# dongzhuoyao/uspace

Hardware: AMD Instinct MI355X
Metric: images/sec, U-ViT-L 256 latent FM sampling (50 ODE steps, bs64) @1/2/4/8 GPU (higher is better)
Workload: dtype bf16

## Files before the change

include/uspace_hip.h:

```cpp
#ifndef USPACE_HIP_H
#define USPACE_HIP_H

#include <stddef.h>
#include <stdint.h>

#ifdef __cplusplus
extern "C" {
#endif

#define USPACE_ABI_VERSION 11

#define USPACE_OK 0
#define USPACE_ERR_ARG (-1)
#define USPACE_ERR_LAUNCH (-2)
#define USPACE_ERR_WORKSPACE (-3)

typedef void* uspace_stream_t;

#define USPACE_API __attribute__((visibility("default")))

USPACE_API int uspace_abi_version(void);


#define USPACE_EPI_BIAS 1
// ... 21 lines not shown
    const float* colsum;
    float* c_out;
    int norm_dim;
    float eps;
    const float* row_add;
    const float* col_add;
    void* split_ws;
    size_t split_ws_bytes;
    void* sk_ws;
    size_t sk_ws_bytes;
    void* sk_counters;
} uspace_gemm_ext;
USPACE_API size_t uspace_gemm_split_ws_bytes(int M, int N, int K);
USPACE_API size_t uspace_gemm_sk_ws_bytes(int M, int N, int K);
#define USPACE_GEMM_SK_COUNTERS 256
USPACE_API int uspace_gemm_set_sk(int mode);
USPACE_API int uspace_gemm_get_sk(void);
USPACE_API int uspace_gemm_bf16_ext(const uint16_t* A, int lda, const uint16_t* A2, int lda2, int K1,
                                    const uint16_t* W, int ldw, int M, int N, int K, int epi_flags,
                                    const float* bias, const float* resid_in, int ld_resid,
                                    float* out_f32, int ld_f32, uint16_t* out_bf16, int ld_bf16,
                                    const uspace_gemm_ext* ext, uspace_stream_t stream);
USPACE_API int uspace_fold_layernorm(const float* W, const float* gamma, const float* beta, const float* bias, uint16_t* Wf,
                                     float* bias_out, float* colsum, int N, int K, uspace_stream_t stream);
USPACE_API int uspace_center_rows(const float* x, uint16_t* xc, float* c, float* part, int M, int D, uspace_stream_t stream);
USPACE_API int uspace_uvit_set_ln_fold(int mode);
USPACE_API int uspace_uvit_get_ln_fold(void);
USPACE_API int uspace_gemm_part_slots(int M, int N);
USPACE_API int uspace_gemm_part_slots_k(int M, int N, int K);

USPACE_API int uspace_gemm_tile_choice(int M, int N, int* split_rows);
USPACE_API int uspace_gemm_plan(int M, int N, int* out);
USPACE_API int uspace_gemm_plan_k(int M, int N, int K, int producer, int* out);

USPACE_API int uspace_gemm_slabs_bf16(const uint16_t* A, int lda, const uint16_t* W, int ldw, int M, int N, int K1,
                                      int n_slab, const int* row_shift, int epi_flags, const float* bias,
                                      const float* resid_in, int ld_resid, float* out_f32, int ld_f32,
                                      uint16_t* out_bf16, int ld_bf16, uspace_stream_t stream);

USPACE_API int uspace_layernorm_f32_bf16(const float* x, const float* gamma, const float* beta, uint16_t* y,
                              int M, int D, float eps, uspace_stream_t stream);

USPACE_API int uspace_attention_bf16(const uint16_t* qkv, const float* key_scale, uint16_t* out,
                          int B, int L, int H, uspace_stream_t stream);
USPACE_API int uspace_attention_plan(int B, int L, int H, int scaled, int* out);

USPACE_API int uspace_attention_long_bf16(const uint16_t* qkv, const float* key_scale, uint16_t* out,
                                          int B, int L, int H, uspace_stream_t stream);
USPACE_API int uspace_attention_long_plan(int B, int L, int H, int scaled, int* out);

USPACE_API int uspace_attention_wide_bf16(const uint16_t* q, const uint16_t* k, const uint16_t* v, int ld,
                                          uint16_t* out, int ld_out, int B, int N, int C, float scale,
                                          uspace_stream_t stream);
USPACE_API int uspace_attention_wide_plan(int B, int N, int C, int* out);

USPACE_API int uspace_attention_map_bf16(const uint16_t* qkv, float* out, int B, int L, int H,
                                         int q0, int nq, int k0, int nk, uspace_stream_t stream);

USPACE_API int uspace_embed_tokens(const float* img, const float* t, int t_stride, const float* extra, int n_extra,
                        int time_first, const float* patch_w, const float* patch_b, const float* pos,
                        float* tok, uint16_t* tok_bf16, int B, int C, int S, int p, int D,
                        uspace_stream_t stream);

USPACE_API int uspace_output_head(const float* tok, int L, int extras, const float* norm_g, const float* norm_b,
                       const float* dec_w, const float* dec_b, const float* conv_w, const float* conv_b,
                       float* scratch, float* out, int B, int C, int S, int p, int D, float eps,
// ... 301 lines not shown
```

uspace_amd/_hip.py:

```python
import ctypes
import os

import torch

_HERE = os.path.dirname(os.path.abspath(__file__))
_DEFAULT_LIB = os.path.join(_HERE, "libuspace_hip.so")
LIB_PATH = os.environ.get("USPACE_HIP_LIB") or _DEFAULT_LIB

EPI_BIAS, EPI_GELU, EPI_RESIDUAL, EPI_OUT_F32, EPI_OUT_BF16 = 1, 2, 4, 8, 16
EPI_CEN_OUT, EPI_LN_IN, EPI_RANK1 = 32, 64, 128

ABI_VERSION = 11

_ERR = {-1: "USPACE_ERR_ARG", -2: "USPACE_ERR_LAUNCH", -3: "USPACE_ERR_WORKSPACE"}


class UspaceHipError(RuntimeError):
    pass


class UvitConfig(ctypes.Structure):
    _fields_ = [(n, ctypes.c_int) for n in (
        "img_size", "patch_size", "in_chans", "embed_dim", "depth", "num_heads", "mlp_hidden",
        "n_extra", "clip_dim", "time_first")]
# ... 31 lines not shown
    _fields_ = [("input_size", ctypes.c_int), ("blocks", ctypes.c_int * 4), ("se", ctypes.c_int)]


class GemmExt(ctypes.Structure):
    _fields_ = [("row_c", ctypes.c_void_p), ("out_cen", ctypes.c_void_p), ("ld_cen", ctypes.c_int),
                ("part_out", ctypes.c_void_p), ("part_in", ctypes.c_void_p), ("np_in", ctypes.c_int),
                ("colsum", ctypes.c_void_p), ("c_out", ctypes.c_void_p), ("norm_dim", ctypes.c_int), ("eps", ctypes.c_float),
                ("row_add", ctypes.c_void_p), ("col_add", ctypes.c_void_p),
                ("split_ws", ctypes.c_void_p), ("split_ws_bytes", ctypes.c_size_t),
                ("sk_ws", ctypes.c_void_p), ("sk_ws_bytes", ctypes.c_size_t), ("sk_counters", ctypes.c_void_p)]


_P, _I, _L, _F, _SZ = ctypes.c_void_p, ctypes.c_int, ctypes.c_long, ctypes.c_float, ctypes.c_size_t
_D = ctypes.c_double

SIGNATURES = {
    "uspace_abi_version": (_I, []),
    "uspace_gemm_bf16": (_I, [_P, _I, _P, _I, _I, _P, _I, _I, _I, _I, _I, _P, _P, _I, _P, _I, _P, _I, _P]),
    "uspace_gemm_bf16_ext": (_I, [_P, _I, _P, _I, _I, _P, _I, _I, _I, _I, _I, _P, _P, _I, _P, _I, _P, _I,
                                  ctypes.POINTER(GemmExt), _P]),
    "uspace_gemm_part_slots": (_I, [_I, _I]),
    "uspace_gemm_part_slots_k": (_I, [_I, _I, _I]),
    "uspace_gemm_split_ws_bytes": (_SZ, [_I, _I, _I]),
    "uspace_gemm_sk_ws_bytes": (_SZ, [_I, _I, _I]),
    "uspace_gemm_set_sk": (_I, [_I]),
    "uspace_gemm_get_sk": (_I, []),
    "uspace_fold_layernorm": (_I, [_P, _P, _P, _P, _P, _P, _P, _I, _I, _P]),
    "uspace_center_rows": (_I, [_P, _P, _P, _P, _I, _I, _P]),
    "uspace_uvit_set_ln_fold": (_I, [_I]),
    "uspace_uvit_get_ln_fold": (_I, []),
    "uspace_gemm_tile_choice": (_I, [_I, _I, ctypes.POINTER(_I)]),
    "uspace_gemm_plan": (_I, [_I, _I, ctypes.POINTER(_I)]),
    "uspace_gemm_plan_k": (_I, [_I, _I, _I, _I, ctypes.POINTER(_I)]),
    "uspace_gemm_slabs_bf16": (_I, [_P, _I, _P, _I, _I, _I, _I, _I, ctypes.POINTER(_I), _I, _P, _P, _I, _P, _I, _P, _I, _P]),
    "uspace_layernorm_f32_bf16": (_I, [_P, _P, _P, _P, _I, _I, _F, _P]),
    "uspace_attention_bf16": (_I, [_P, _P, _P, _I, _I, _I, _P]),
    "uspace_attention_plan": (_I, [_I, _I, _I, _I, ctypes.POINTER(_I)]),
    "uspace_attention_long_bf16": (_I, [_P, _P, _P, _I, _I, _I, _P]),
    "uspace_attention_long_plan": (_I, [_I, _I, _I, _I, ctypes.POINTER(_I)]),
    "uspace_attention_wide_bf16": (_I, [_P, _P, _P, _I, _P, _I, _I, _I, _I, _F, _P]),
    "uspace_attention_wide_plan": (_I, [_I, _I, _I, ctypes.POINTER(_I)]),
    "uspace_attention_map_bf16": (_I, [_P, _P, _I, _I, _I, _I, _I, _I, _I, _P]),
    "uspace_embed_tokens": (_I, [_P, _P, _I, _P, _I, _I, _P, _P, _P, _P, _P, _I, _I, _I, _I, _I, _P]),
    "uspace_output_head": (_I, [_P, _I, _I, _P, _P, _P, _P, _P, _P, _P, _P, _I, _I, _I, _I, _I, _F, _P]),
    "uspace_add_broadcast": (_I, [_P, _P, _P, _F, _I, _L, _P]),
    "uspace_add_broadcast_rows": (_I, [_P, _P, _P, _F, _P, _I, _L, _P]),
    "uspace_cast_f32_bf16": (_I, [_P, _P, _L, _P]),
    "uspace_cfg_combine": (_I, [_P, _P, _F, _P, _I, _L, _P]),
    "uspace_direction_accumulate": (_I, [_P, _P, _P, _P, _I, _L, _I, _P]),
    "uspace_center_cols_f32": (_I, [_P, _P, _I, _L, _P]),
    "uspace_gram_f64": (_I, [_P, _P, _I, _L, _P]),
    "uspace_project_rows_f64": (_I, [_P, _P, _P, _I, _I, _L, _P]),
    "uspace_normalize_rows_signed": (_I, [_P, _I, _L, _P]),
    "uspace_ode_combine": (_I, [_P, _P, ctypes.POINTER(_P), ctypes.POINTER(_F), _I, _L, _P]),
    "uspace_ode_error_norm": (_I, [_P, _P, ctypes.POINTER(_P), ctypes.POINTER(_F), _I, _F, _F, _L, _P, _P, _P]),
    "uspace_uvit_num_params": (_I, [ctypes.POINTER(UvitConfig)]),
    "uspace_uvit_param_numel": (_L, [ctypes.POINTER(UvitConfig), _I]),
    "uspace_uvit_weight_bytes": (_SZ, [ctypes.POINTER(UvitConfig)]),
    "uspace_uvit_workspace_bytes": (_SZ, [ctypes.POINTER(UvitConfig), _I]),
    "uspace_uvit_pack_weights": (_I, [ctypes.POINTER(UvitConfig), ctypes.POINTER(_P), _I, _P, _SZ, _P]),
    "uspace_uvit_forward": (_I, [ctypes.POINTER(UvitConfig), _P, _P, _SZ, ctypes.POINTER(UvitIO), _I, _P]),
    "uspace_uvit_forward_maps": (_I, [ctypes.POINTER(UvitConfig), _P, _P, _SZ, ctypes.POINTER(UvitIO), _I, _I, _I, _I, _I, _P, _P]),
    "uspace_uvit_cfg_workspace_bytes": (_SZ, [ctypes.POINTER(UvitConfig), _I]),
    "uspace_uvit_forward_cfg": (_I, [ctypes.POINTER(UvitConfig), _P, _P, _SZ, ctypes.POINTER(UvitIO), _I, _P, _I, _F, _P, _P, _P]),
    "uspace_uvit_forward_tap": (_I, [ctypes.POINTER(UvitConfig), _P, _P, _SZ, ctypes.POINTER(UvitIO), _I, _I, _P, _P]),
    "uspace_uvit_graph_create": (_I, [ctypes.POINTER(UvitConfig), _P, _P, _SZ, ctypes.POINTER(UvitIO), _I, _P,
# ... 483 lines not shown
```

uspace_amd/csrc/gemm.hip:

```cpp
#include <algorithm>
#include <atomic>
#include <type_traits>
#include <vector>

#include "common.h"
#include "gemm_args.h"

namespace {

using namespace usgemm;


#ifndef USPACE_LAB
#define USPACE_LAB 0
#endif
constexpr size_t sk_slab_bytes(int BM, int BN, bool xtra) { return (size_t)((BM / 16) * (BN / 16) + (xtra ? BN / 16 : 0)) * 1024; }
constexpr double TALL_COST = 0.60;
constexpr int ROW_BYTES = 128;

template <int WM, int XN, int TN>
__device__ __forceinline__ bf16x8 pick_w(const bf16x8 (&wf)[TN], int wm, int j) {
    if constexpr (WM == 4) {
        const bf16x8 a = wf[j], b = wf[XN + j], c = wf[2 * XN + j], d = wf[3 * XN + j];
        const bf16x8 lo = (wm & 1) ? b : a, hi = (wm & 1) ? d : c;
// ... 7 lines not shown

template <int WM, int XN, int TN>
__device__ __forceinline__ f32x4 pick_b(const f32x4 (&b)[TN], int wm, int j) {
    if constexpr (WM == 4) {
        const f32x4 a = b[j], b1 = b[XN + j], c = b[2 * XN + j], d = b[3 * XN + j];
        const f32x4 lo = (wm & 1) ? b1 : a, hi = (wm & 1) ? d : c;
        return (wm & 2) ? hi : lo;
    }
    f32x4 r = b[j];
#pragma unroll
    for (int w = 1; w < WM; ++w) r = (wm == w) ? b[w * XN + j] : r;
    return r;
}

__device__ __forceinline__ uint4 widen_pair(uint2 a, uint2 b) {
    const auto rx = __builtin_amdgcn_permlane16_swap(a.x, b.x, false, false);
    const auto ry = __builtin_amdgcn_permlane16_swap(a.y, b.y, false, false);
    return make_uint4(rx[0], ry[0], rx[1], ry[1]);
}

__device__ __forceinline__ int lds_off(int r, int c) { return r * ROW_BYTES + ((c ^ ((r >> 1) & 7)) << 4); }

template <int N>
__device__ __forceinline__ void wait_vm() {
    asm volatile("s_waitcnt vmcnt(%0) lgkmcnt(0)" ::"n"(N) : "memory");
}

constexpr int stage_bytes(int BM, int BN, bool xtra) { return (BM + BN + (xtra ? 16 : 0)) * ROW_BYTES; }
constexpr int rowv_bytes(int BM, int flags) { return (flags & (USPACE_EPI_LN_IN | USPACE_EPI_CEN_OUT)) ? (BM + 16) * 8 : 0; }
__device__ __forceinline__ int strip_of_tile_row(int tile_m, int tiles_m) {
    return (tiles_m & 7) == 0 ? (tile_m & 7) * (tiles_m >> 3) + (tile_m >> 3) : tile_m;
}

template <int BM, int BN, int WM, int WN, int FLAGS, bool XTRA, int NST, bool SK, bool OWNER>
__device__ __forceinline__ void gemm_tile(const GemmArgs& g, char* const smem, const int tile_m, const int tile_n, const int sk_tile,
                                          const int sk_split) {
    static_assert(!OWNER || (XTRA && NST == 2 && !SK), "a strip owner's body has the strips and is a two-stage whole-tile form");
    constexpr int THREADS = 64 * WM * WN;
    constexpr int TM = BM / WM / 16;
    constexpr int TN = BN / WN / 16;
    constexpr int HM = TM / 2;
    constexpr int XN = TN / WM;
    constexpr int ROWS_PER_ISSUE = THREADS / 8;
    constexpr int ISSUES_A = BM / ROWS_PER_ISSUE;
    constexpr int ISSUES_W = BN / ROWS_PER_ISSUE;
    constexpr int TILE_A_BYTES = BM * ROW_BYTES;
    constexpr int TILE_W_BYTES = BN * ROW_BYTES;
    constexpr int TILE_X_BYTES = XTRA ? 16 * ROW_BYTES : 0;
    constexpr int STAGE_BYTES = TILE_A_BYTES + TILE_W_BYTES + TILE_X_BYTES;
    static_assert(BM % ROWS_PER_ISSUE == 0 && BN % ROWS_PER_ISSUE == 0, "tile/threads mismatch");
    static_assert(TM % 2 == 0 && TN % WM == 0 && (WM == 2 || WM == 4), "wave tile shape");
    static_assert(NST == 2 || (!XTRA && FLAGS == USPACE_EPI_OUT_F32) || (BM == 64 && BN == 64),
                  "the ring form: raw fp32 partial sums of a K range (K-split), or the 64 x 64 tiles with any epilogue");
    constexpr int IPT = ISSUES_A + ISSUES_W;
    static_assert((NST - 1) * IPT < 64, "vmcnt is a 6-bit counter");
    static_assert(!SK || (NST == 2 && WM * WN == 8), "the in-launch K-split tail is written for the 8-wave two-stage forms (one workgroup per CU)");

    constexpr bool ROWV = (FLAGS & (USPACE_EPI_LN_IN | USPACE_EPI_CEN_OUT)) != 0;
    static_assert(STAGE_BYTES == stage_bytes(BM, BN, XTRA), "the kernel sizes the LDS object with stage_bytes");
    const uint32_t rowv_lds = (uint32_t)(uintptr_t)(US_LDS char*)(smem + NST * STAGE_BYTES);

    const int tid = threadIdx.x;
    const int lane = tid & 63;
    const int wave = __builtin_amdgcn_readfirstlane(tid >> 6);
    const int wm = wave / WN;
    const int wn = wave % WN;

    const int m0 = tile_m * BM;
    const int n0 = tile_n * BN;
    const int m_lim = XTRA ? g.m_main : g.M;
    const int sk = strip_of_tile_row(tile_m, g.tiles_m);
    const int x0 = g.m_main + sk * 16;
    const int xr = (XTRA && sk < g.n_strip) ? (g.M - x0 < 16 ? g.M - x0 : 16) : 0;
    const bool has_x = OWNER || xr > 0;

    const int srow = tid >> 3;
    const int schunk = tid & 7;
    const bf16_t* const gA = g.A;
    const bf16_t* const gA2 = g.A2;
    const bf16_t* const gW = g.W;
    uint32_t a_off[ISSUES_A];
    uint32_t w_off[ISSUES_W];
#pragma unroll
    for (int i = 0; i < ISSUES_A; ++i) {
        const int r = i * ROWS_PER_ISSUE + srow;
        const int c = schunk ^ ((r >> 1) & 7);
        int m = m0 + r;
        m = m < m_lim ? m : m_lim - 1;
        a_off[i] = (uint32_t)(m * g.lda + c * 8) * 2u;
    }
#pragma unroll
    for (int i = 0; i < ISSUES_W; ++i) {
        const int r = i * ROWS_PER_ISSUE + srow;
        const int c = schunk ^ ((r >> 1) & 7);
        int n = n0 + r;
        n = n < g.N ? n : g.N - 1;
        w_off[i] = (uint32_t)(n * g.ldw + c * 8) * 2u;
    }
    uint32_t x_off = 0;
    if constexpr (XTRA) {
        const int r = tid >> 3;
        const int c = schunk ^ ((r >> 1) & 7);
        int m = x0 + (r < xr ? r : 0);
        m = m < g.M ? m : g.M - 1;
        x_off = (uint32_t)(m * g.lda + c * 8) * 2u;
    }
    const int wave_lds_off = wave * 8 * ROW_BYTES;
// ... 28 lines not shown
        char* base = smem + buf * STAGE_BYTES + TILE_A_BYTES;
        const __amdgpu_buffer_rsrc_t rs = __builtin_amdgcn_make_buffer_rsrc((void*)wbase, 0, 0x7fffffff, 0x00020000);
#pragma unroll
        for (int i = 0; i < ISSUES_W; ++i) dma16(rs, w_off[i], base + i * ROWS_PER_ISSUE * ROW_BYTES + wave_lds_off);
    };

    const int fr = lane & 15;
    const int fq = lane >> 4;
    const int a_lds = (wm * (BM / WM) + fr) * ROW_BYTES;
    const int w_lds = TILE_A_BYTES + (wn * (BN / WN) + fr) * ROW_BYTES;
    const int x_lds = TILE_A_BYTES + TILE_W_BYTES + fr * ROW_BYTES;
    const int swz = (fr >> 1) & 7;
    const int c_k0 = ((fq) ^ swz) << 4;
    const int c_k1 = ((4 + fq) ^ swz) << 4;

    f32x4 acc[TM][TN];
    f32x4 xacc[XTRA ? XN : 1];
    if ((FLAGS & USPACE_EPI_RESIDUAL) != 0 && (!SK || sk_split == 0)) {
#pragma unroll
        for (int i = 0; i < TM; ++i) {
            int m = m0 + wm * (BM / WM) + i * 16 + fr;
            m = m < m_lim ? m : m_lim - 1;
#pragma unroll
            for (int j = 0; j < TN; ++j) {
                int n = n0 + wn * (BN / WN) + j * 16 + fq * 4;
                n = n < g.N ? n : g.N - 4;
                acc[i][j] = *(const f32x4*)(g.resid + (size_t)m * g.ld_resid + n);
            }
        }
        if constexpr (XTRA) {
            int m = x0 + (fr < xr ? fr : 0);
            m = m < g.M ? m : g.M - 1;
#pragma unroll
            for (int j = 0; j < XN; ++j) {
                int n = n0 + wn * (BN / WN) + (wm * XN + j) * 16 + fq * 4;
                n = n < g.N ? n : g.N - 4;
                xacc[j] = *(const f32x4*)(g.resid + (size_t)m * g.ld_resid + n);
            }
        }
    } else {
#pragma unroll
        for (int i = 0; i < TM; ++i)
#pragma unroll
            for (int j = 0; j < TN; ++j) acc[i][j] = (f32x4){0.f, 0.f, 0.f, 0.f};
#pragma unroll
        for (int j = 0; j < (XTRA ? XN : 1); ++j) xacc[j] = (f32x4){0.f, 0.f, 0.f, 0.f};
    }

    bf16x8 af0[HM], af1[HM], wf0[TN], wf1[TN], xf0, xf1;

    constexpr bool LN_IN = (FLAGS & USPACE_EPI_LN_IN) != 0, CEN = (FLAGS & USPACE_EPI_CEN_OUT) != 0;
    constexpr bool RK1 = (FLAGS & USPACE_EPI_RANK1) != 0;
    static_assert(!RK1 || (CEN && !LN_IN), "the rank-1 term belongs to a LayerNorm producer (skip_linear)");
    constexpr bool CSV = LN_IN || RK1;
    constexpr bool EARLY_EPI = BM * BN <= 256 * 128;
    f32x4 bias4[TN];
    f32x4 cs4[CSV ? TN : 1];
    auto load_epi_consts = [&]() {
        if constexpr (FLAGS & USPACE_EPI_BIAS) {
#pragma unroll
            for (int j = 0; j < TN; ++j) {
                int n = n0 + wn * (BN / WN) + j * 16 + fq * 4;
                n = n < g.N ? n : g.N - 4;
                bias4[j] = *(const f32x4*)(g.bias + n);
            }
        }
        if constexpr (CSV) {
            const float* const cv = RK1 ? g.col_add : g.colsum;
#pragma unroll
            for (int j = 0; j < TN; ++j) {
                int n = n0 + wn * (BN / WN) + j * 16 + fq * 4;
                n = n < g.N ? n : g.N - 4;
                cs4[j] = *(const f32x4*)(cv + n);
            }
        }
    };

#define LOAD_A(dst, base, mh, ck)                                                                   \
    _Pragma("unroll") for (int i_ = 0; i_ < HM; ++i_)                                               \
        dst[i_] = *(const bf16x8*)((base) + a_lds + ((mh) * HM + i_) * 16 * ROW_BYTES + (ck));
#define LOAD_W(dst, base, ck)                                                                       \
    _Pragma("unroll") for (int j_ = 0; j_ < TN; ++j_)                                               \
        dst[j_] = *(const bf16x8*)((base) + w_lds + j_ * 16 * ROW_BYTES + (ck));
#define LOAD_X(dst, base, ck) if (X_ON) dst = *(const bf16x8*)((base) + x_lds + (ck));
#define MMA(af, wf, mh, ilo, ihi)                                                                   \
    _Pragma("unroll") for (int i_ = (ilo); i_ < (ihi); ++i_)                                        \
        _Pragma("unroll") for (int jj_ = 0; jj_ < TN; ++jj_) {                                      \
            const int j_ = (i_ & 1) ? TN - 1 - jj_ : jj_;                                           \
            acc[(mh) * HM + i_][j_] =                                                               \
                __builtin_amdgcn_mfma_f32_16x16x32_bf16(wf[j_], af[i_], acc[(mh) * HM + i_][j_], 0, 0, 0); \
        }
#define MMA_X(xf, wf)                                                                               \
    if (XTRA && X_ON) {                                                                             \
        _Pragma("unroll") for (int j_ = 0; j_ < XN; ++j_)                                           \
            xacc[j_] = __builtin_amdgcn_mfma_f32_16x16x32_bf16(pick_w<WM, XN>(wf, wm, j_), xf, xacc[j_], 0, 0, 0); \
    }

    const bool X_ON = has_x;
    const int nk = NST > 2 ? g.nk_split : (SK && sk_tile >= 0) ? (sk_split + 1) * (g.K / BK) / g.sk_S - kt0 : g.K / BK;
    float2 pr[ROWV ? 8 : 1];
    float rc_v = 0.f, ra_v = 0.f;
    int rv_m = -1;
    auto fetch_rowv = [&]() {
        static_assert(BM + 16 <= THREADS || !ROWV, "one thread per tile row");
        const int t = tid;
        if (t < BM + (XTRA ? 16 : 0)) {
            const bool strip = t >= BM;
            const int m = strip ? x0 + (t - BM) : m0 + t;
            const bool ok = strip ? ((t - BM) < xr && m < g.M) : (m < m_lim);
            if (ok) {
                rv_m = m;
                if constexpr ((FLAGS & USPACE_EPI_LN_IN) != 0) {
#pragma unroll
                    for (int q = 0; q < 8; ++q)
                        pr[q] = q < g.np_in ? *(const float2*)(g.part_in + ((size_t)m * g.np_in + q) * 2) : make_float2(0.f, 0.f);
                    if (n0 == 0 && g.c_out && sk_split == 0) rc_v = g.row_c[m];
                } else {
                    rc_v = g.row_c[m];
                    if constexpr (RK1) ra_v = g.row_add[m];
                }
            }
        }
    };
    if constexpr (NST > 2) {
        if constexpr (ROWV) fetch_rowv();
        if constexpr (EARLY_EPI) load_epi_consts();
#pragma unroll
        for (int t = 0; t < 2; ++t) {
            stage_a(t, t, has_x);
            stage_w(t, t);
        }
        wait_vm<IPT>();
        __builtin_amdgcn_s_barrier();
#pragma unroll
        for (int t = 2; t < NST; ++t) {
            stage_a(t, t, has_x);
            stage_w(t, t);
        }
    } else {
        stage_a(0, 0, has_x);
        stage_w(0, 0);
        if (nk > 1) stage_a(1, 1, has_x);
        if constexpr (ROWV) fetch_rowv();
        if constexpr (EARLY_EPI) load_epi_consts();
        __syncthreads();
    }
    if constexpr (ROWV) {
        if (tid < BM + (XTRA ? 16 : 0)) {
            float2 v = make_float2(0.f, 1.f);
            if (rv_m >= 0) {
                if constexpr ((FLAGS & USPACE_EPI_LN_IN) != 0) {
                    float s1 = 0.f, s2 = 0.f;
#pragma unroll
                    for (int q = 0; q < 8; ++q) {
                        s1 += pr[q].x;
                        s2 += pr[q].y;
                    }
                    const float d = s1 * g.inv_d;
                    v = make_float2(d, rsqrtf(fmaxf(s2 * g.inv_d - d * d, 0.f) + g.eps));
                    if (n0 == 0 && g.c_out && sk_split == 0) g.c_out[rv_m] = rc_v + d;
                } else {
                    v = make_float2(rc_v, ra_v);
                }
            }
            asm volatile("ds_write_b64 %0, %1" ::"v"(rowv_lds + (uint32_t)tid * 8u), "v"(v) : "memory");
        }
    }
    constexpr bool TINYK = NST > 2 && BM == 64 && BN == 64;
    if constexpr (!TINYK) {
        LOAD_A(af0, smem, 0, c_k0)
        LOAD_W(wf0, smem, c_k0)
        if constexpr (XTRA) { LOAD_X(xf0, smem, c_k0) }
    }

    constexpr bool EARLYB = BM == 256 && BN == 128;
#define KTILE(kt, MORE, MORE2)                                                                     \
    {                                                                                              \
        const char* cur = smem + (kt & 1) * STAGE_BYTES;                                           \
        MMA(af0, wf0, 0, 0, 1)                                                                     \
        MMA_X(xf0, wf0)                                                                            \
        __builtin_amdgcn_sched_barrier(0);                                                         \
        if (MORE) stage_w(kt + 1, (kt + 1) & 1);                                                   \
        LOAD_A(af1, cur, 1, c_k0)                                                                  \
        __builtin_amdgcn_sched_barrier(0);                                                         \
        MMA(af0, wf0, 0, 1, HM)                                                                    \
        __builtin_amdgcn_sched_barrier(0);                                                         \
        MMA(af1, wf0, 1, 0, 1)                                                                     \
        __builtin_amdgcn_sched_barrier(0);                                                         \
        LOAD_A(af0, cur, 0, c_k1)                                                                  \
        LOAD_W(wf1, cur, c_k1)                                                                     \
        if constexpr (XTRA) { LOAD_X(xf1, cur, c_k1) }                                             \
        __builtin_amdgcn_sched_barrier(0);                                                         \
        MMA(af1, wf0, 1, 1, HM)                                                                    \
// ... 149 lines not shown
        KTILE_TT(0) KTILE_TT(1) KTILE_TT(2) KTILE_TT(3) KTILE_TT(4) KTILE_TT(5) KTILE_TT(6)
#undef KTILE_TT
        static_assert(NST <= 8, "tail steps are written out up to NST = 8");
        T_MMA((NST - 1) & 1)
#undef KTILE_T
#undef T_MMA
#undef T_LOAD
    } else if constexpr (NST > 2) {
        int kt = 0, buf = 0;
        for (; kt + NST < nk; ++kt) {
            const int nb = buf + 1 == NST ? 0 : buf + 1;
            KTILE_R(kt, buf, nb, true, true, (NST - 2) * IPT)
            buf = nb;
        }
#define KTILE_TAIL(J)                                                                              \
        if constexpr ((J) < NST - 1) {                                                             \
            const int nb = buf + 1 == NST ? 0 : buf + 1;                                           \
            KTILE_R(kt, buf, nb, true, false, (NST - 2 - (J)) * IPT)                               \
            buf = nb;                                                                              \
            ++kt;                                                                                  \
        }
        KTILE_TAIL(0) KTILE_TAIL(1) KTILE_TAIL(2) KTILE_TAIL(3) KTILE_TAIL(4) KTILE_TAIL(5) KTILE_TAIL(6)
#undef KTILE_TAIL
        static_assert(NST <= 8, "tail steps are written out up to NST = 8");
        KTILE_R(kt, buf, 0, false, false, 0)
    } else {
        auto kloop = [&](auto xon) __attribute__((always_inline)) {
            constexpr bool X_ON = decltype(xon)::value;
            int kt = 0;
            for (; kt + 2 < nk; ++kt) KTILE(kt, true, true)
            if (kt + 1 < nk) { KTILE(kt, true, false) ++kt; }
            KTILE(kt, false, false)
        };
        if constexpr (OWNER) {
            kloop(std::true_type{});
        } else if constexpr (XTRA && (FLAGS & USPACE_EPI_RESIDUAL) == 0) {
            if (has_x) kloop(std::true_type{});
            else kloop(std::false_type{});
        } else if constexpr (XTRA) {
            int kt = 0;
            for (; kt + 2 < nk; ++kt) KTILE(kt, true, true)
            if (kt + 1 < nk) { KTILE(kt, true, false) ++kt; }
            KTILE(kt, false, false)
        } else {
            kloop(std::false_type{});
        }
    }
#undef KTILE_R
#undef KTILE
#undef LOAD_A
#undef LOAD_W
#undef LOAD_X
#undef MMA
#undef MMA_X

    int own_lo = 0, own_hi = TM;
    if constexpr (SK) {
        if (sk_tile >= 0) {
            const int S = g.sk_S;
            own_lo = sk_split * TM / S;
            own_hi = (sk_split + 1) * TM / S;
            constexpr int WSLOTS = TM * TN + (XTRA ? XN : 0);
            constexpr size_t SLAB_BYTES = (size_t)WM * WN * WSLOTS * 1024;
            static_assert(SLAB_BYTES == sk_slab_bytes(BM, BN, XTRA), "host and kernel agree on the slab size");
            char* const slabs = (char*)g.sk_ws + (size_t)sk_tile * S * SLAB_BYTES;
            const uint32_t lane_off = (uint32_t)(wave * WSLOTS) * 1024u + (uint32_t)lane * 16u;
            typedef __attribute__((ext_vector_type(4))) unsigned u32x4_t;
// ... 197 lines not shown
                    pc[j].x = pack_bf2(vc[0], vc[1]);
                    pc[j].y = pack_bf2(vc[2], vc[3]);
                }
            }
            if constexpr (CEN) {
                ps1 = (s1v[0] + s1v[1]) + (s1v[2] + s1v[3]);
                ps2 = (s2v[0] + s2v[1]) + (s2v[2] + s2v[3]);
            }
#pragma unroll
            for (int j = 0; j < TN; j += 2) {
                if constexpr (FLAGS & USPACE_EPI_OUT_BF16) *(uint4*)(g.out_bf16 + (size_t)m * g.ld_bf16 + nw + j * 16) = widen_pair(pk[j], pk[j + 1]);
                if constexpr (CEN) *(uint4*)(g.out_cen + (size_t)m * g.ld_cen + nw + j * 16) = widen_pair(pc[j], pc[j + 1]);
            }
            row_end(m, true, wm * (BM / WM) + i * 16 + fr, wn);
        }
    } else {
#pragma unroll
        for (int i = 0; i < TM; ++i) {
            if (SK && (i < own_lo || i >= own_hi)) continue;
            const int m = m0 + wm * (BM / WM) + i * 16 + fr;
            const bool vrow = m < m_lim;
            row_begin(i);
            if (vrow) {
#pragma unroll
                for (int j = 0; j < TN; ++j) {
                    const int n = n0 + wn * (BN / WN) + j * 16 + fq * 4;
                    if (n >= g.N) continue;
                    emit(acc[i][j], bias4[j], m, n, cs4[CSV ? j : 0]);
                }
            }
            row_end(m, vrow, wm * (BM / WM) + i * 16 + fr, wn);
        }
    }
    if constexpr (OWNER && !CEN) {
        static_assert(!OWNER || XN % 2 == 0, "the strip's sub-tiles are widened in pairs");
        const int m = x0 + fr;
        const bool vrow = fr < xr;
        row_begin(TM);
        f32x4 v[XN];
#pragma unroll
        for (int j = 0; j < XN; ++j) {
            f32x4 csx = cs4[0];
            if constexpr (CSV) csx = pick_b<WM, XN>(cs4, wm, j);
            v[j] = emit_pre(xacc[j], pick_b<WM, XN>(bias4, wm, j), csx);
        }
        if constexpr (FLAGS & USPACE_EPI_GELU) gelu_erf_batch<XN>(v);
        const int nx = n0 + wn * (BN / WN) + wm * XN * 16;
        if (n0 + BN <= g.N && g.wide) {
            uint2 pk[XN];
#pragma unroll
            for (int j = 0; j < XN; ++j) {
                if constexpr (FLAGS & USPACE_EPI_OUT_BF16) {
                    pk[j].x = pack_bf2(v[j][0], v[j][1]);
                    pk[j].y = pack_bf2(v[j][2], v[j][3]);
                }
            }
            uint4 wk[XN / 2];
#pragma unroll
            for (int j = 0; j < XN; j += 2) {
                if constexpr (FLAGS & USPACE_EPI_OUT_BF16) wk[j / 2] = widen_pair(pk[j], pk[j + 1]);
            }
            if (vrow) {
                const int nw = nx + (fq & 1) * 16 + (fq >> 1) * 8;
#pragma unroll
                for (int j = 0; j < XN; ++j)
                    if constexpr ((FLAGS & USPACE_EPI_OUT_F32) != 0) *(f32x4*)(out_f32 + (size_t)m * g.ld_f32 + nx + j * 16 + fq * 4) = v[j];
#pragma unroll
// ... 22 lines not shown
                    if constexpr (CSV) csx = pick_b<WM, XN>(cs4, wm, j);
                    emit(xacc[j], pick_b<WM, XN>(bias4, wm, j), m, n, csx);
                }
            }
        }
        row_end(m, vrow, BM + fr, wm == 0 ? wn : -(wm * WN + wn) - 1);
    }
    if constexpr (CEN) {
        __syncthreads();
        for (int t = tid; t < BM + (XTRA ? 16 : 0); t += THREADS) {
            const bool strip = t >= BM;
            const int m = strip ? x0 + (t - BM) : m0 + t;
            bool ok = strip ? ((t - BM) < xr && m < g.M) : (m < m_lim);
            if constexpr (SK) {
                const int it = (t % (BM / WM)) >> 4;
                ok = ok && (strip ? own_x : (it >= own_lo && it < own_hi));
            }
            if (!ok) continue;
            float a = 0.f, bq = 0.f;
            const int nslot = strip ? RSLOTS : WN;
#pragma unroll 1
            for (int q = 0; q < nslot; ++q) {
                a += red[(t * RSLOTS + q) * 2];
                bq += red[(t * RSLOTS + q) * 2 + 1];
            }
            float* po = g.part_out + ((size_t)m * g.tiles_n + n0 / BN) * 2;
            po[0] = a;
            po[1] = bq;
        }
    }
}

constexpr bool role_bodies(int BM, int BN, bool xtra, int nst, bool sk) { return xtra && BM == 256 && BN == 256 && nst == 2 && !sk; }

template <int BM, int BN, int WM, int WN, int FLAGS, bool XTRA, int NST = 2, bool SK = false>
__global__ __launch_bounds__(64 * WM * WN, (WM * WN == 4 && (NST == 2 || BM == 64)) ? 2 : 1) void gemm_kernel(const GemmArgs g) {
    __shared__ __attribute__((aligned(16))) char smem[NST * stage_bytes(BM, BN, XTRA) + rowv_bytes(BM, FLAGS)];
    const int nwg = g.tiles_m * g.tiles_n;
    int tile_m, tile_n;
    int sk_tile = -1, sk_split = 0;
    {
        int b = blockIdx.x;
        if constexpr (SK) {
            if (b >= g.sk_first) {
                const int u = b - g.sk_first, v = u >> 3;
                sk_split = v % g.sk_S;
                sk_tile = (v / g.sk_S) * 8 + (u & 7);
                b = g.sk_first + sk_tile;
                if (b >= nwg) return;
            }
        }
        const int xcd = b & 7, idx = b >> 3;
        const int n_super = nwg >> 5;
        if ((g.tiles_m & 7) == 0 && (g.tiles_n & 3) == 0 && (n_super & 7) == 0) {
            const int mb_count = g.tiles_m >> 3;
            const int sup = xcd + 8 * (idx >> 5);
            const int t = idx & 31;
            tile_m = (sup % mb_count) * 8 + (t >> 2);
            tile_n = (sup / mb_count) * 4 + (t & 3);
        } else {
            const int q = nwg >> 3, r = nwg & 7;
            const int tile = (xcd < r ? xcd * (q + 1) : r * (q + 1) + (xcd - r) * q) + idx;
            tile_m = tile / g.tiles_n;
            tile_n = tile % g.tiles_n;
        }
    }
    if constexpr (role_bodies(BM, BN, XTRA, NST, SK)) {
        if (strip_of_tile_row(tile_m, g.tiles_m) < g.n_strip) gemm_tile<BM, BN, WM, WN, FLAGS, true, NST, SK, true>(g, smem, tile_m, tile_n, sk_tile, sk_split);
        else gemm_tile<BM, BN, WM, WN, FLAGS, false, NST, SK, false>(g, smem, tile_m, tile_n, sk_tile, sk_split);
    } else {
        gemm_tile<BM, BN, WM, WN, FLAGS, XTRA, NST, SK, false>(g, smem, tile_m, tile_n, sk_tile, sk_split);
    }
}

enum TileChoice { TILE_BIG = 0, TILE_MID = 1, TILE_SMALL = 2, TILE_SPLIT = 3, TILE_TALL = 4, TILE_TINY = 5, TILE_SK = 6 };
constexpr int TINY_SLOTS = 1024, TINY_RING_SLOTS = 512;
struct TileShape { int BM, BN, WM, WN, per_round; };
constexpr TileShape SHAPES[] = {
    {256, 256, 2, 4, 256},
    {192, 256, 2, 4, 256},
    {128, 128, 2, 2, 512},
    {256, 256, 2, 4, 256},
    {256, 128, 4, 2, 256},
    {64, 64, 2, 2, TINY_SLOTS},
    {256, 256, 2, 4, 256},
};

template <TileChoice F, int FLAGS, int NST = 2>
int launch(const GemmArgs& a, hipStream_t s, const Plan& p) {
    constexpr TileShape t = SHAPES[F];
    GemmArgs g = a;
    if constexpr (NST > 2) {
        g.nk_split = g.K / BK;
        g.split_stride = 0;
    }
    g.tiles_n = us_cdiv(g.N, t.BN);
    g.tiles_m = p.tiles_m;
    g.m_main = p.m_main;
    g.n_strip = p.n_strip;
    const int rec = us_rec_begin(US_REC_GEMM, FLAGS, g.M, g.N, g.K, s);
    const dim3 grid(g.tiles_m * g.tiles_n), block(64 * t.WM * t.WN);
    if (p.n_strip > 0) hipLaunchKernelGGL((gemm_kernel<t.BM, t.BN, t.WM, t.WN, FLAGS, true, NST>), grid, block, 0, s, g);
    else hipLaunchKernelGGL((gemm_kernel<t.BM, t.BN, t.WM, t.WN, FLAGS, false, NST>), grid, block, 0, s, g);
    us_rec_end(rec, s);
    US_CHECK_LAUNCH();
    return USPACE_OK;
}

struct SkPlan {
    Plan rows;
    int tiles_n, n_dp, n_sk, groups, S;
};
#if USPACE_LAB && defined(USPACE_SK_MIN_NK)
constexpr int SK_MIN_NK = USPACE_SK_MIN_NK, SK_MIN_KT = USPACE_SK_MIN_KT;
#else
constexpr int SK_MIN_NK = 64;
constexpr int SK_MIN_KT = 16;
#endif
constexpr double SK_FIXED = 0.10;
std::atomic<int> g_sk_on{1};
inline bool sk_plan(int M, int N, int K, SkPlan* out) {
    if (M < 256 || N < 256 || (N & 255) || K % BK || K / BK < SK_MIN_NK) return false;
    const int tn = N / 256, tm = M / 256, rem = M - tm * 256, nk = K / BK;
    SkPlan p;
    p.tiles_n = tn;
    if (rem == 0) p.rows = Plan{tm, M, 0};
    else if (rem <= 16 * tm) p.rows = Plan{tm, tm * 256, us_cdiv(rem, 16)};
    else p.rows = Plan{tm + 1, M, 0};
    const int T = p.rows.tiles_m * tn;
    p.n_dp = T / 256 * 256;
    p.n_sk = T - p.n_dp;
    if (p.n_sk == 0) return false;
// ... 364 lines not shown
extern "C" int uspace_gemm_part_slots(int M, int N) { return uspace_gemm_part_slots_k(M, N, BK); }

extern "C" size_t uspace_gemm_split_ws_bytes(int M, int N, int K) {
    if (M <= 0 || N <= 0 || K <= 0) return 0;
    const GemmPlan p = plan_gemm(M, N, K, false, false, true);
    return p.split_k > 1 ? (size_t)p.split_k * M * N * 4 : 0;
}

extern "C" int uspace_gemm_tile_choice(int M, int N, int* split_rows) {
    if (M <= 0 || N <= 0) return USPACE_ERR_ARG;
    const GemmPlan p = plan_gemm(M, N, BK, false, false, true);
    if (split_rows) *split_rows = p.split_rows;
    return (int)p.form;
}

static void format_plan(const GemmPlan& p, int* out) {
    const bool sk = p.form == TILE_SK;
    out[0] = (int)p.form; out[1] = sk ? p.sk.S : p.split_rows; out[2] = p.shape.BM; out[3] = p.shape.BN;
    out[4] = p.rows.tiles_m; out[5] = p.tiles_n; out[6] = p.rows.n_strip; out[7] = sk ? p.sk.n_dp : p.shape.per_round;
}

extern "C" int uspace_gemm_plan(int M, int N, int* out) {
    if (M <= 0 || N <= 0 || !out) return USPACE_ERR_ARG;
    format_plan(plan_gemm(M, N, BK, false, false, true), out);
    return USPACE_OK;
}

extern "C" int uspace_gemm_plan_k(int M, int N, int K, int producer, int* out) {
    if (M <= 0 || N <= 0 || K <= 0 || !out) return USPACE_ERR_ARG;
    format_plan(plan_gemm(M, N, K, producer != 0, g_sk_on.load(std::memory_order_relaxed) != 0), out);
    return USPACE_OK;
}

size_t us_gemm_sk_ws_bytes(int M, int N, int K, bool sk_on) {
    if (M <= 0 || N <= 0 || K <= 0) return 0;
    size_t need = 0;
    for (int producer = 0; producer < 2; ++producer) {
        const GemmPlan p = plan_gemm(M, N, K, producer != 0, sk_on);
        if (p.form == TILE_SK) need = std::max(need, sk_ws_need(p.sk));
    }
    return need;
}
extern "C" size_t uspace_gemm_sk_ws_bytes(int M, int N, int K) { return us_gemm_sk_ws_bytes(M, N, K, g_sk_on.load(std::memory_order_relaxed) != 0); }

int us_gemm_bf16_ext(const uint16_t* A, int lda, const uint16_t* A2, int lda2, int K1, const uint16_t* W, int ldw, int M, int N, int K,
                     int epi_flags, const float* bias, const float* resid_in, int ld_resid, float* out_f32, int ld_f32, uint16_t* out_bf16,
                     int ld_bf16, const uspace_gemm_ext* ext, bool sk_on, uspace_stream_t stream) {
    GemmArgs g;
    US_TRY(plain_args(g, A, lda, W, ldw, M, N, K, K1, epi_flags, bias, resid_in, ld_resid, out_f32, ld_f32, out_bf16, ld_bf16));
    g.lda2 = lda2;
    if (K1 < K) {
        if (!A2 || lda2 != lda || K != 2 * K1 || (K1 & (K1 - 1))) return USPACE_ERR_ARG;
        g.A2 = A2;
        g.n_slab = 2;
        while ((1 << g.k1_log2) < K1) ++g.k1_log2;
    }
    if (ext) {
        g.split_ws = (float*)ext->split_ws; g.split_ws_bytes = ext->split_ws_bytes;
        if (g.split_ws && ((uintptr_t)g.split_ws & 15)) return USPACE_ERR_ARG;
        if (ext->sk_ws && ext->sk_counters) {
            if (((uintptr_t)ext->sk_ws & 15) || ((uintptr_t)ext->sk_counters & 3)) return USPACE_ERR_ARG;
            g.sk_ws = (float*)ext->sk_ws; g.sk_ws_bytes = ext->sk_ws_bytes; g.sk_cnt = (unsigned*)ext->sk_counters;
        }
        g.row_c = ext->row_c; g.out_cen = ext->out_cen; g.ld_cen = ext->ld_cen; g.part_out = ext->part_out;
        g.part_in = ext->part_in; g.np_in = ext->np_in; g.colsum = ext->colsum; g.c_out = ext->c_out;
        g.row_add = ext->row_add; g.col_add = ext->col_add;
// ... 51 lines not shown
```

uspace_amd/csrc/gemm_args.h:

```cpp
#pragma once
#include "common.h"

namespace usgemm {

struct GemmArgs {
    const bf16_t* A;
    const bf16_t* A2;
    const bf16_t* W;
    const float* bias;
    const float* resid;
    float* out_f32;
    bf16_t* out_bf16;
    int M, N, K, K1;
    int lda, lda2, ldw, ld_resid, ld_f32, ld_bf16;
    int tiles_m, tiles_n;
    int n_slab, k1_log2;
    int slab_shift[9];
    int m_main, n_strip;
    const float* row_c;
    bf16_t* out_cen;
    float* part_out;
    const float* part_in;
    const float* colsum;
    float* c_out;
    const float* row_add;
    const float* col_add;
    int ld_cen, np_in;
    float inv_d, eps;
    int wide;
    int nk_split;
    long split_stride;
    float* split_ws;
    size_t split_ws_bytes;
    int sk_first, sk_S;
    float* sk_ws;
    unsigned* sk_cnt;
    size_t sk_ws_bytes;
};

constexpr int BK = 64;

struct Plan {
    int tiles_m, m_main, n_strip;
};

inline double strip_factor(const Plan& p, int BM) {
    if (p.n_strip <= 0) return 1.0;
    return 1.0 + ((double)p.n_strip / p.tiles_m) * (16.0 / BM) + 0.01;
}

inline Plan plan_rows(int M, int BM, int tiles_n, int wg_per_round) {
// ... 20 lines not shown
```

Baseline: 20.63.

## Spread leftover-row strip work across sixteen tiles instead of one owner

For 256x256 two-stage GEMMs with residual epilogues, the leftover 16-row strip is now shared across sixteen main tiles. Each sharer tile has one extra wave compute a single 16-column subtile of the strip, instead of one owner tile computing the whole strip. The aim is to even out per-workgroup work so the owner tile no longer makes the grid's tail longer. The cost is an extra template body, a new argument field, a query API, and a guard on the c_out writes.

Result: no change. 20.62, median of 2 (-0.0%).

```diff
diff --git a/include/uspace_hip.h b/include/uspace_hip.h
--- a/include/uspace_hip.h
+++ b/include/uspace_hip.h
@@ -77,6 +77,7 @@
 USPACE_API int uspace_gemm_tile_choice(int M, int N, int* split_rows);
 USPACE_API int uspace_gemm_plan(int M, int N, int* out);
 USPACE_API int uspace_gemm_plan_k(int M, int N, int K, int producer, int* out);
+USPACE_API int uspace_gemm_strip_share(int M, int N, int K, int epi_flags);
 
 USPACE_API int uspace_gemm_slabs_bf16(const uint16_t* A, int lda, const uint16_t* W, int ldw, int M, int N, int K1,
                                       int n_slab, const int* row_shift, int epi_flags, const float* bias,
diff --git a/uspace_amd/_hip.py b/uspace_amd/_hip.py
--- a/uspace_amd/_hip.py
+++ b/uspace_amd/_hip.py
@@ -87,6 +87,7 @@
     "uspace_gemm_tile_choice": (_I, [_I, _I, ctypes.POINTER(_I)]),
     "uspace_gemm_plan": (_I, [_I, _I, ctypes.POINTER(_I)]),
     "uspace_gemm_plan_k": (_I, [_I, _I, _I, _I, ctypes.POINTER(_I)]),
+    "uspace_gemm_strip_share": (_I, [_I, _I, _I, _I]),
     "uspace_gemm_slabs_bf16": (_I, [_P, _I, _P, _I, _I, _I, _I, _I, ctypes.POINTER(_I), _I, _P, _P, _I, _P, _I, _P, _I, _P]),
     "uspace_layernorm_f32_bf16": (_I, [_P, _P, _P, _P, _I, _I, _F, _P]),
     "uspace_attention_bf16": (_I, [_P, _P, _P, _I, _I, _I, _P]),
diff --git a/uspace_amd/csrc/gemm.hip b/uspace_amd/csrc/gemm.hip
--- a/uspace_amd/csrc/gemm.hip
+++ b/uspace_amd/csrc/gemm.hip
@@ -63,10 +63,12 @@
     return (tiles_m & 7) == 0 ? (tile_m & 7) * (tiles_m >> 3) + (tile_m >> 3) : tile_m;
 }
 
-template <int BM, int BN, int WM, int WN, int FLAGS, bool XTRA, int NST, bool SK, bool OWNER>
+template <int BM, int BN, int WM, int WN, int FLAGS, bool XTRA, int NST, bool SK, bool OWNER, bool SHARER = false>
 __device__ __forceinline__ void gemm_tile(const GemmArgs& g, char* const smem, const int tile_m, const int tile_n, const int sk_tile,
                                           const int sk_split) {
     static_assert(!OWNER || (XTRA && NST == 2 && !SK), "a strip owner's body has the strips and is a two-stage whole-tile form");
+    static_assert(!SHARER || (XTRA && NST == 2 && !SK && !OWNER && (FLAGS & USPACE_EPI_CEN_OUT) == 0 && BN / WN / 16 == 4),
+                  "a sharer's body: two-stage whole-tile form, no partial sums, four column sub-tiles per wave");
     constexpr int THREADS = 64 * WM * WN;
     constexpr int TM = BM / WM / 16;
     constexpr int TN = BN / WN / 16;
@@ -100,10 +102,12 @@
     const int m0 = tile_m * BM;
     const int n0 = tile_n * BN;
     const int m_lim = XTRA ? g.m_main : g.M;
-    const int sk = strip_of_tile_row(tile_m, g.tiles_m);
+    const int sk = SHARER ? tile_m >> 4 : strip_of_tile_row(tile_m, g.tiles_m);
     const int x0 = g.m_main + sk * 16;
     const int xr = (XTRA && sk < g.n_strip) ? (g.M - x0 < 16 ? g.M - x0 : 16) : 0;
-    const bool has_x = OWNER || xr > 0;
+    const bool has_x = OWNER || SHARER || xr > 0;
+    const int xq = tile_m & 15, xj = xq & 3;
+    const bool is_sh = SHARER && wave == WN + (xq >> 2);
 
     const int srow = tid >> 3;
     const int schunk = tid & 7;
@@ -198,8 +202,8 @@
             int m = x0 + (fr < xr ? fr : 0);
             m = m < g.M ? m : g.M - 1;
 #pragma unroll
-            for (int j = 0; j < XN; ++j) {
-                int n = n0 + wn * (BN / WN) + (wm * XN + j) * 16 + fq * 4;
+            for (int j = 0; j < (SHARER ? 1 : XN); ++j) {
+                int n = n0 + (SHARER ? xq * 16 : wn * (BN / WN) + (wm * XN + j) * 16) + fq * 4;
                 n = n < g.N ? n : g.N - 4;
                 xacc[j] = *(const f32x4*)(g.resid + (size_t)m * g.ld_resid + n);
             }
@@ -248,7 +252,7 @@
 #define LOAD_W(dst, base, ck)                                                                       \
     _Pragma("unroll") for (int j_ = 0; j_ < TN; ++j_)                                               \
         dst[j_] = *(const bf16x8*)((base) + w_lds + j_ * 16 * ROW_BYTES + (ck));
-#define LOAD_X(dst, base, ck) if (X_ON) dst = *(const bf16x8*)((base) + x_lds + (ck));
+#define LOAD_X(dst, base, ck) if (X_ON && (!SHARER || is_sh)) dst = *(const bf16x8*)((base) + x_lds + (ck));
 #define MMA(af, wf, mh, ilo, ihi)                                                                   \
     _Pragma("unroll") for (int i_ = (ilo); i_ < (ihi); ++i_)                                        \
         _Pragma("unroll") for (int jj_ = 0; jj_ < TN; ++jj_) {                                      \
@@ -257,7 +261,9 @@
                 __builtin_amdgcn_mfma_f32_16x16x32_bf16(wf[j_], af[i_], acc[(mh) * HM + i_][j_], 0, 0, 0); \
         }
 #define MMA_X(xf, wf)                                                                               \
-    if (XTRA && X_ON) {                                                                             \
+    if constexpr (SHARER) {                                                                         \
+        if (is_sh) xacc[0] = __builtin_amdgcn_mfma_f32_16x16x32_bf16(pick_w<4, 1>(wf, xj, 0), xf, xacc[0], 0, 0, 0); \
+    } else if (XTRA && X_ON) {                                                                      \
         _Pragma("unroll") for (int j_ = 0; j_ < XN; ++j_)                                           \
             xacc[j_] = __builtin_amdgcn_mfma_f32_16x16x32_bf16(pick_w<WM, XN>(wf, wm, j_), xf, xacc[j_], 0, 0, 0); \
     }
@@ -324,7 +330,7 @@
                     }
                     const float d = s1 * g.inv_d;
                     v = make_float2(d, rsqrtf(fmaxf(s2 * g.inv_d - d * d, 0.f) + g.eps));
-                    if (n0 == 0 && g.c_out && sk_split == 0) g.c_out[rv_m] = rc_v + d;
+                    if (n0 == 0 && g.c_out && sk_split == 0 && (!SHARER || tid < BM || xq == 0)) g.c_out[rv_m] = rc_v + d;
                 } else {
                     v = make_float2(rc_v, ra_v);
                 }
@@ -540,7 +546,7 @@
             if (kt + 1 < nk) { KTILE(kt, true, false) ++kt; }
             KTILE(kt, false, false)
         };
-        if constexpr (OWNER) {
+        if constexpr (OWNER || SHARER) {
             kloop(std::true_type{});
         } else if constexpr (XTRA && (FLAGS & USPACE_EPI_RESIDUAL) == 0) {
             if (has_x) kloop(std::true_type{});
@@ -804,7 +810,15 @@
             row_end(m, vrow, wm * (BM / WM) + i * 16 + fr, wn);
         }
     }
-    if constexpr (OWNER && !CEN) {
+    if constexpr (SHARER) {
+        const int m = x0 + fr, n = n0 + xq * 16 + fq * 4;
+        row_begin(TM);
+        if (is_sh && fr < xr && n < g.N) {
+            f32x4 csx = cs4[0];
+            if constexpr (CSV) csx = pick_b<4, 1>(cs4, xj, 0);
+            emit(xacc[0], pick_b<4, 1>(bias4, xj, 0), m, n, csx);
+        }
+    } else if constexpr (OWNER && !CEN) {
         static_assert(!OWNER || XN % 2 == 0, "the strip's sub-tiles are widened in pairs");
         const int m = x0 + fr;
         const bool vrow = fr < xr;
@@ -893,6 +907,11 @@
 }
 
 constexpr bool role_bodies(int BM, int BN, bool xtra, int nst, bool sk) { return xtra && BM == 256 && BN == 256 && nst == 2 && !sk; }
+
+constexpr bool sharer_flags(int f) {
+    constexpr int B_ = USPACE_EPI_BIAS, R_ = USPACE_EPI_RESIDUAL, F_ = USPACE_EPI_OUT_F32, H_ = USPACE_EPI_OUT_BF16;
+    return f == (B_ | R_ | F_ | H_) || f == (B_ | R_ | F_);
+}
 
 template <int BM, int BN, int WM, int WN, int FLAGS, bool XTRA, int NST = 2, bool SK = false>
 __global__ __launch_bounds__(64 * WM * WN, (WM * WN == 4 && (NST == 2 || BM == 64)) ? 2 : 1) void gemm_kernel(const GemmArgs g) {
@@ -927,7 +946,15 @@
         }
     }
     if constexpr (role_bodies(BM, BN, XTRA, NST, SK)) {
-        if (strip_of_tile_row(tile_m, g.tiles_m) < g.n_strip) gemm_tile<BM, BN, WM, WN, FLAGS, true, NST, SK, true>(g, smem, tile_m, tile_n, sk_tile, sk_split);
+        int role = strip_of_tile_row(tile_m, g.tiles_m) < g.n_strip ? 1 : 0;
+        if constexpr (sharer_flags(FLAGS)) {
+            if (g.share) role = tile_m < g.n_strip * 16 ? 2 : 0;
+            if (role == 2) {
+                gemm_tile<BM, BN, WM, WN, FLAGS, true, NST, SK, false, true>(g, smem, tile_m, tile_n, sk_tile, sk_split);
+                return;
+            }
+        }
+        if (role == 1) gemm_tile<BM, BN, WM, WN, FLAGS, true, NST, SK, true>(g, smem, tile_m, tile_n, sk_tile, sk_split);
         else gemm_tile<BM, BN, WM, WN, FLAGS, false, NST, SK, false>(g, smem, tile_m, tile_n, sk_tile, sk_split);
     } else {
         gemm_tile<BM, BN, WM, WN, FLAGS, XTRA, NST, SK, false>(g, smem, tile_m, tile_n, sk_tile, sk_split);
@@ -947,6 +974,10 @@
     {256, 256, 2, 4, 256},
 };
 
+constexpr bool strip_share(int BM, int BN, int nst, int flags, const Plan& p) {
+    return role_bodies(BM, BN, p.n_strip > 0, nst, false) && sharer_flags(flags) && p.n_strip * 16 <= p.tiles_m;
+}
+
 template <TileChoice F, int FLAGS, int NST = 2>
 int launch(const GemmArgs& a, hipStream_t s, const Plan& p) {
     constexpr TileShape t = SHAPES[F];
@@ -959,6 +990,7 @@
     g.tiles_m = p.tiles_m;
     g.m_main = p.m_main;
     g.n_strip = p.n_strip;
+    g.share = strip_share(t.BM, t.BN, NST, FLAGS, p) ? 1 : 0;
     const int rec = us_rec_begin(US_REC_GEMM, FLAGS, g.M, g.N, g.K, s);
     const dim3 grid(g.tiles_m * g.tiles_n), block(64 * t.WM * t.WN);
     if (p.n_strip > 0) hipLaunchKernelGGL((gemm_kernel<t.BM, t.BN, t.WM, t.WN, FLAGS, true, NST>), grid, block, 0, s, g);
@@ -1389,6 +1421,13 @@
     return USPACE_OK;
 }
 
+extern "C" int uspace_gemm_strip_share(int M, int N, int K, int epi_flags) {
+    if (M <= 0 || N <= 0 || K <= 0) return USPACE_ERR_ARG;
+    const GemmPlan p = plan_gemm(M, N, K, (epi_flags & USPACE_EPI_CEN_OUT) != 0, g_sk_on.load(std::memory_order_relaxed) != 0 && sk_flags(epi_flags));
+    if (p.form != TILE_BIG && p.form != TILE_SPLIT) return 0;
+    return strip_share(p.shape.BM, p.shape.BN, p.nst, epi_flags, p.rows) ? 1 : 0;
+}
+
 size_t us_gemm_sk_ws_bytes(int M, int N, int K, bool sk_on) {
     if (M <= 0 || N <= 0 || K <= 0) return 0;
     size_t need = 0;
diff --git a/uspace_amd/csrc/gemm_args.h b/uspace_amd/csrc/gemm_args.h
--- a/uspace_amd/csrc/gemm_args.h
+++ b/uspace_amd/csrc/gemm_args.h
@@ -17,6 +17,7 @@
     int n_slab, k1_log2;
     int slab_shift[9];
     int m_main, n_strip;
+    int share;
     const float* row_c;
     bf16_t* out_cen;
     float* part_out;
```
